# tencent-ailab/V-Express

Hardware: NVIDIA H100
Metric: frames_per_sec_512x512_25step (higher is better)
Workload: dtype bf16

## Files before the change

v-express_b200/csrc/vx_gemm.cu:

```cuda
#include "vx_host.h"
#include "vx_ptx.cuh"

namespace vx {

constexpr int kBlockM = 128;
constexpr int kBlockK = 64;
constexpr int kThreads = 384;
constexpr int kEpiThreads = 256;
constexpr int kPPMaxBN = 96;
constexpr int kPanelCols = 32;
constexpr int kPanelBytes = kBlockM * kPanelCols * 2;
constexpr int kSmemCap = 227 * 1024;
constexpr int kSmemReserve = 2048;

struct GemmArgs {
  int M, N;
  int kblocks1;
  int kblocks2;
  int taps;
  int rr;
  int a_bytes;
  int ups;
  int block_n;
  int pp;
  int stages;
  int nbuf;
  int rows_valid;
  int W, H;
  int cstride;
  int cpad;
  int tiles_m, tiles_n;
  int geglu;
  int has_residual;
  int out_f32;
  const float* bias;
  const float* bias2;
  int bias2_div;
  float scale;
  float* out32;
  long long ldc;
  const float* ln_stats;
  const float* ln_colsum;
  int ares;
  int ares_bytes;
  float2* rs_out;
  long long rs_stride;
  const float2* ln_parts;
  long long ln_pstride;
  int ln_nparts;
  float ln_invK;
  float ln_eps;
};

__device__ __forceinline__ void tma_store_2d(const CUtensorMap* m, const void* src, int c0, int c1) {
  asm volatile("cp.async.bulk.tensor.2d.global.shared::cta.bulk_group [%0, {%2, %3}], [%1];" ::"l"(
                   reinterpret_cast<uint64_t>(m)),
               "r"(smem_u32(src)), "r"(c0), "r"(c1)
               : "memory");
}
__device__ __forceinline__ void tma_store_5d(const CUtensorMap* m, const void* src, int c0, int c1, int c2, int c3, int c4) {
  asm volatile("cp.async.bulk.tensor.5d.global.shared::cta.bulk_group [%0, {%2, %3, %4, %5, %6}], [%1];" ::"l"(
                   reinterpret_cast<uint64_t>(m)),
// ... 45 lines not shown
  uint8_t* ring = smem;
  if constexpr (LNF) ring += p.ares ? p.ares_bytes : 0;
  uint8_t* sC = ring + p.stages * stage_bytes;
  const int out_cols = p.geglu ? BN / 2 : BN;
  const int npanels = out_cols / kPanelCols;
  const int buf_bytes = npanels * kPanelBytes;
  uint64_t* full_bar = reinterpret_cast<uint64_t*>(sC + (p.out_f32 ? 0 : p.nbuf * buf_bytes));
  uint64_t* empty_bar = full_bar + p.stages;
  uint64_t* c_ready = empty_bar + p.stages;
  uint64_t* staged = c_ready + 2;
  uint64_t* a_land = staged + 2;
  uint64_t* a_empty = a_land + 8;

  const int warp = threadIdx.x >> 5;
  const int lane = threadIdx.x & 31;
  const int total_kb = p.rr ? 3 * p.kblocks1 : p.taps * p.kblocks1 + p.kblocks2;
  const int tiles_per_par = p.tiles_m * p.tiles_n;
  const int num_tiles = tiles_per_par * (p.ups ? 4 : 1);
  auto item_at = [&](int it) -> int {
    if constexpr (LNF) {
      if (p.ares) {
        const int g = (int)blockIdx.x + (it / p.tiles_n) * (int)gridDim.x;
        return g < p.tiles_m ? g * p.tiles_n + it % p.tiles_n : -1;
      }
    }
    const int t = (int)blockIdx.x + it * (int)gridDim.x;
    return t < num_tiles ? t : -1;
  };

  if (threadIdx.x == 0) {
    tma_prefetch_desc(&mapA);
    tma_prefetch_desc(&mapB);
    if (p.kblocks2) tma_prefetch_desc(&mapA2);
    if (!p.out_f32) tma_prefetch_desc(&mapC);
    if (p.has_residual || p.ups) tma_prefetch_desc(&mapR);
    constexpr int consumers = PP ? kEpiThreads / 2 : kEpiThreads;
    for (int s = 0; s < p.stages; ++s) {
      mbar_init(&full_bar[s], 1);
      mbar_init(&empty_bar[s], consumers / 32);
    }
    for (int s = 0; s < 2; ++s) {
      mbar_init(&c_ready[s], 1);
      mbar_init(&staged[s], consumers);
    }
    for (int s = 0; s < 8; ++s) {
      mbar_init(&a_land[s], 1);
      mbar_init(&a_empty[s], kEpiThreads / 32);
    }
    fence_barrier_init();
  }
  __syncthreads();
  pdl_wait();

  if (warp < 4) setmaxnreg_dec<40>();
  else setmaxnreg_inc<232>();

  if (warp == 0) {
    const bool leader = elect_one();
    int stage = 0;
    uint32_t phase = 0;
    for (int it = 0, t = item_at(0); t >= 0; t = item_at(++it)) {
      const int par = t / tiles_per_par, tt = t - par * tiles_per_par;
      const int tile_n = tt % p.tiles_n, tile_m = tt / p.tiles_n;
      int n0 = 0, y0 = 0, x0 = 0;
      const long long m0 = (long long)tile_m * p.rows_valid;
      if (p.taps != 1) {
        const long long hw = (long long)p.H * p.W;
        n0 = (int)(m0 / hw);
        const int rem = (int)(m0 % hw);
        y0 = rem / p.W;
        x0 = rem % p.W;
      }
      const uint32_t tx_bytes = (uint32_t)((p.rr ? a_bytes : p.rows_valid * kBlockK * 2) + nbt * b_bytes);
      const int b_row = par * p.N + tile_n * BN;
      if constexpr (LNF) {
        if (p.ares && tile_n == 0) {
          for (int kb = 0; kb < p.kblocks1; ++kb) {
            mbar_wait(&a_empty[kb], (uint32_t)(((it / p.tiles_n) & 1) ^ 1));
            if (leader) {
              mbar_expect_tx(&a_land[kb], (uint32_t)(kBlockM * kBlockK * 2));
              tma_load_2d(smem + kb * (kBlockM * kBlockK * 2), &mapA, &a_land[kb], kb * kBlockK, (int)m0);
            }
          }
          __syncwarp();
        }
      }
      for (int kb = 0; kb < total_kb; ++kb) {
        mbar_wait(&empty_bar[stage], phase ^ 1);
        uint8_t* sa = ring + stage * stage_bytes;
        uint8_t* sb = sa + a_bytes;
        const int tap = p.taps != 1 ? kb / p.kblocks1 : 0;
        const int cb = kb - tap * p.kblocks1;
        if constexpr (LNF) {
          if (p.ares) {
            if (leader) {
              mbar_expect_tx(&full_bar[stage], (uint32_t)b_bytes);
              tma_load_2d(ring + stage * stage_bytes, &mapB, &full_bar[stage], kb * kBlockK, b_row);
            }
            __syncwarp();
            if (++stage == p.stages) {
              stage = 0;
              phase ^= 1;
            }
            continue;
          }
        }
        if (leader) {
          mbar_expect_tx(&full_bar[stage], tx_bytes);
          if (p.rr) {
            tma_load_4d(sa, &mapA, &full_bar[stage], cb * kBlockK, x0 + tap - 1, y0 - 1, n0);
#pragma unroll
            for (int dyi = 0; dyi < 3; ++dyi)
              tma_load_2d(sb + dyi * b_bytes, &mapB, &full_bar[stage], ((dyi * 3 + tap) * p.kblocks1 + cb) * kBlockK, b_row);
          } else {
            const int dy = p.ups ? (tap >> 1) + (par >> 1) - 1 : tap / 3 - p.cpad;
            const int dx = p.ups ? (tap & 1) + (par & 1) - 1 : tap % 3 - p.cpad;
            if (p.taps != 1) {
              tma_load_4d(sa, &mapA, &full_bar[stage], cb * kBlockK, x0 * p.cstride + dx, y0 * p.cstride + dy, n0);
            } else if (kb < p.kblocks1) {
              tma_load_2d(sa, &mapA, &full_bar[stage], kb * kBlockK, (int)m0);
            } else {
              tma_load_2d(sa, &mapA2, &full_bar[stage], (kb - p.kblocks1) * kBlockK, (int)m0);
            }
            tma_load_2d(sb, &mapB, &full_bar[stage], kb * kBlockK, b_row);
          }
        }
        __syncwarp();
        if (++stage == p.stages) {
          stage = 0;
          phase ^= 1;
        }
      }
    }
  } else if (warp == 1) {
    if (lane == 0 && !p.out_f32) {
      const uint32_t res_bytes = (uint32_t)(p.rows_valid * out_cols * 2);
      auto arm = [&](int t, int b) {
        if (p.has_residual) {
          const int tn_ = t % p.tiles_n, tm_ = t / p.tiles_n;
          mbar_expect_tx(&c_ready[b], res_bytes);
          for (int pn = 0; pn < npanels; ++pn)
            tma_load_2d(sC + b * buf_bytes + pn * kPanelBytes, &mapR, &c_ready[b], tn_ * out_cols + pn * kPanelCols,
                        tm_ * p.rows_valid);
        } else {
          mbar_arrive(&c_ready[b]);
        }
      };
      for (int b = 0; b < p.nbuf; ++b)
        if (item_at(b) >= 0) arm(item_at(b), b);
      for (int it = 0, t = item_at(0); t >= 0; t = item_at(++it)) {
        const int b = it % p.nbuf;
        const int par = t / tiles_per_par, tt = t - par * tiles_per_par;
        const int tile_n = tt % p.tiles_n, tile_m = tt / p.tiles_n;
        mbar_wait(&staged[b], (uint32_t)((it / p.nbuf) & 1));
        if (p.ups) {
          const long long m0 = (long long)tile_m * p.rows_valid, hw = (long long)p.H * p.W;
          const int n0 = (int)(m0 / hw), rem = (int)(m0 % hw);
          const CUtensorMap* mo = (par & 1) ? &mapR : &mapC;
          if (m0 < p.M)
            for (int pn = 0; pn < npanels; ++pn)
              tma_store_5d(mo, sC + b * buf_bytes + pn * kPanelBytes, tile_n * out_cols + pn * kPanelCols, rem % p.W,
                           rem / p.W, n0, par >> 1);
        } else {
          for (int pn = 0; pn < npanels; ++pn)
            tma_store_2d(&mapC, sC + b * buf_bytes + pn * kPanelBytes, tile_n * out_cols + pn * kPanelCols,
                         tile_m * p.rows_valid);
        }
        tma_store_commit();
        const int tnext = item_at(it + p.nbuf);
        if (tnext >= 0) {
          tma_store_wait_read();
          arm(tnext, b);
        }
      }
      tma_store_wait_all();
    }
  } else if (warp >= 4) {
    static_assert(!(PP && LNF) && (!PP || BN <= kPPMaxBN), "ping-pong: plain epilogues, BN <= 96");
    constexpr int MH = PP ? 2 : 1;
    const int wg = (threadIdx.x >> 7) - 1;
    const int wrow = (PP ? 0 : wg * 64) + (warp & 3) * 16 + (lane >> 2);
    const int cq = (lane & 3) * 2;
    float acc[MH][BN / 2];
#pragma unroll
    for (int mh = 0; mh < MH; ++mh)
#pragma unroll
      for (int i = 0; i < BN / 2; ++i) acc[mh][i] = 0.f;
    float ln_mean[2] = {0.f, 0.f}, ln_rstd[2] = {1.f, 1.f};
    for (int it = PP ? wg : 0, t = item_at(it); t >= 0; it += PP ? 2 : 1, t = item_at(it)) {
      const long long g0 = (long long)it * total_kb;
      int stage = (int)(g0 % p.stages);
      uint32_t phase = (uint32_t)((g0 / p.stages) & 1);
      if constexpr (PP) {
        if (it > 0) asm volatile("bar.sync %0, 256;" ::"r"(1 + wg) : "memory");
      }
      const int tt = t % tiles_per_par;
      const int tile_n = tt % p.tiles_n, tile_m = tt / p.tiles_n;
      bool a_last = false;
      if constexpr (LNF) {
        if (p.ares) {
          a_last = tile_n == p.tiles_n - 1;
          if (tile_n == 0) {
            const uint32_t a_phase = (uint32_t)((it / p.tiles_n) & 1);
            float s[2] = {0.f, 0.f};
            for (int kb = 0; kb < p.kblocks1; ++kb) {
              mbar_wait(&a_land[kb], a_phase);
#pragma unroll
              for (int h = 0; h < 2; ++h) {
                const uint8_t* rowp = smem + kb * (kBlockM * kBlockK * 2) + (wrow + 8 * h) * 128;
#pragma unroll
                for (int j = 0; j < 2; ++j) {
                  const uint4 q = *reinterpret_cast<const uint4*>(rowp + ((lane & 3) + 4 * j) * 16);
                  const uint32_t w[4] = {q.x, q.y, q.z, q.w};
#pragma unroll
                  for (int i = 0; i < 4; ++i) {
                    const float2 f2 = unpack_bf16(w[i]);
                    s[h] += f2.x + f2.y;
                  }
                }
              }
            }
            const float invK = 1.0f / (float)(p.kblocks1 * kBlockK);
#pragma unroll
            for (int h = 0; h < 2; ++h) ln_mean[h] = quad_sum(s[h]) * invK;
            float q2[2] = {0.f, 0.f};
            for (int kb = 0; kb < p.kblocks1; ++kb) {
#pragma unroll
              for (int h = 0; h < 2; ++h) {
                const uint8_t* rowp = smem + kb * (kBlockM * kBlockK * 2) + (wrow + 8 * h) * 128;
#pragma unroll
                for (int j = 0; j < 2; ++j) {
                  const uint4 q = *reinterpret_cast<const uint4*>(rowp + ((lane & 3) + 4 * j) * 16);
                  const uint32_t w[4] = {q.x, q.y, q.z, q.w};
#pragma unroll
                  for (int i = 0; i < 4; ++i) {
                    const float2 f2 = unpack_bf16(w[i]);
                    const float d0 = f2.x - ln_mean[h], d1 = f2.y - ln_mean[h];
                    q2[h] = fmaf(d0, d0, q2[h]);
                    q2[h] = fmaf(d1, d1, q2[h]);
                  }
                }
              }
            }
#pragma unroll
            for (int h = 0; h < 2; ++h) ln_rstd[h] = rsqrtf(quad_sum(q2[h]) * invK + p.ln_eps);
          }
        }
      }
      int prev = -1;
      for (int kb = 0; kb < total_kb; ++kb) {
        mbar_wait(&full_bar[stage], phase);
        uint32_t sa = smem_u32(ring + stage * stage_bytes);
        const uint32_t sb = sa + (uint32_t)a_bytes;
        if constexpr (LNF) {
          if (p.ares) sa = smem_u32(smem + kb * (kBlockM * kBlockK * 2));
        }
        if constexpr (!PP) sa += (uint32_t)(wg * 64 * 128);
        wgmma_fence();
        if (!PP && p.rr) {
#pragma unroll
          for (int dyi = 0; dyi < 3; ++dyi) {
            const uint64_t da = make_smem_desc(sa + (uint32_t)(dyi * p.W * 128), 16, 1024, SWZ_128B);
            const uint64_t db = make_smem_desc(sb + (uint32_t)(dyi * b_bytes), 16, 1024, SWZ_128B);
#pragma unroll
            for (int k = 0; k < kBlockK / 16; ++k)
              Wgmma<BN>::template ss<0, 0>(acc[0], da + (uint64_t)(k * 2), db + (uint64_t)(k * 2), (kb | dyi | k) != 0);
          }
        } else {
          const uint64_t db = make_smem_desc(sb, 16, 1024, SWZ_128B);
#pragma unroll
          for (int k = 0; k < kBlockK / 16; ++k)
#pragma unroll
            for (int mh = 0; mh < MH; ++mh) {
              const uint64_t da = make_smem_desc(sa + (uint32_t)(mh * 64 * 128), 16, 1024, SWZ_128B);
              Wgmma<BN>::template ss<0, 0>(acc[mh], da + (uint64_t)(k * 2), db + (uint64_t)(k * 2), (kb | k) != 0);
            }
        }
        wgmma_commit();
        wgmma_wait<1>();
        if (prev >= 0 && lane == 0) mbar_arrive(&empty_bar[prev]);
        prev = stage;
        if (++stage == p.stages) {
          stage = 0;
          phase ^= 1;
        }
      }
      if constexpr (PP) {
        if (item_at(it + 1) >= 0) asm volatile("bar.arrive %0, 256;" ::"r"(1 + (wg ^ 1)) : "memory");
      }
      wgmma_wait<0>();
#pragma unroll
      for (int mh = 0; mh < MH; ++mh) wgmma_fence_regs(acc[mh]);
      if (lane == 0) {
        mbar_arrive(&empty_bar[prev]);
        if constexpr (LNF) {
          if (a_last)
            for (int kb = 0; kb < p.kblocks1; ++kb) mbar_arrive(&a_empty[kb]);
        }
      }

      const int sb = it % p.nbuf;
      if (!p.out_f32) mbar_wait(&c_ready[sb], (uint32_t)((it / p.nbuf) & 1));
      uint8_t* buf = sC + sb * buf_bytes;
      const int nbase = tile_n * BN;
#pragma unroll
      for (int mh = 0; mh < MH; ++mh) {
        const int rbase = wrow + 64 * mh;
        float (&ac)[BN / 2] = acc[mh];
        long long m[2];
        bool row_ok[2];
        const float* b2[2];
#pragma unroll
        for (int h = 0; h < 2; ++h) {
          const int r = rbase + 8 * h;
          m[h] = (long long)tile_m * p.rows_valid + r;
          row_ok[h] = r < p.rows_valid && m[h] < p.M;
          b2[h] = p.bias2 ? p.bias2 + (row_ok[h] ? (m[h] / p.bias2_div) : 0) * (long long)p.N : nullptr;
          if constexpr (LNF) {
            if (p.ares) {
// ... 83 lines not shown
                const float2 t2 = unpack_bf16(pk);
                const int half = nl >= BN / 2;
                rs_sum[h][half] += t2.x + t2.y;
                rs_sq[h][half] = fmaf(t2.x, t2.x, fmaf(t2.y, t2.y, rs_sq[h][half]));
              }
            }
          }
          if (!PP && p.rs_out) {
#pragma unroll
            for (int h = 0; h < 2; ++h)
#pragma unroll
              for (int half = 0; half < 2; ++half) {
                const float s1 = quad_sum(rs_sum[h][half]), s2 = quad_sum(rs_sq[h][half]);
                if ((lane & 3) == 0 && row_ok[h]) p.rs_out[(long long)(tile_n * 2 + half) * p.rs_stride + m[h]] = make_float2(s1, s2);
              }
          }
        }
      }
      if (!p.out_f32) {
        fence_proxy_async_smem();
        mbar_arrive(&staged[sb]);
      }
    }
  }
}

struct GemmEnv {
  int stages, nbuf, bn, verbose, conv_rr, pp;
  static int geti(const char* name, int dflt) {
    const char* s = getenv(name);
    return s ? atoi(s) : dflt;
  }
  GemmEnv() {
    stages = geti("VX_GEMM_STAGES", 0);
    nbuf = geti("VX_GEMM_NBUF", 0);
    bn = geti("VX_GEMM_BN", 0);
    verbose = geti("VX_GEMM_VERBOSE", 0);
    conv_rr = geti("VX_CONV_RR", 1);
    pp = geti("VX_GEMM_PP", -1);
  }
};
static GemmEnv& gemm_env() {
  static GemmEnv e;
  return e;
}

static bool bn_supported(int bn) {
  switch (bn) {
    case 16: case 32: case 64: case 96: case 128: case 160: case 192: case 256: return true;
    default: return false;
  }
}

static bool pp_bn_supported(int bn) { return bn == 32 || bn == 64 || bn == 96; }

static int pick_block_n(long long tiles_m, int N, int gran, int total_kb, int fixed_bn = 0, bool pp_ok = false,
                        int* pp = nullptr) {
  const int mode = gemm_env().pp;
  if (pp) *pp = 0;
  if (pp_ok && mode != 0) {
    for (int bn = kPPMaxBN; bn >= 32; bn -= 32) {
      if (mode == -1 && bn != kPPMaxBN) break;
      if (N % bn || bn % gran || (fixed_bn > 0 && bn != fixed_bn)) continue;
      if (pp) *pp = 1;
      return bn;
    }
  }
  const int sms = device_sms();
  int best = 0;
  double best_cost = 1e30;
  for (int bn = 256; bn >= gran; bn -= gran) {
    if (N % bn || !bn_supported(bn) || (fixed_bn > 0 && bn != fixed_bn)) continue;
    const long long items = tiles_m * (N / bn);
    const double waves = (double)((items + sms - 1) / sms);
    const double cyc = (4.0 * bn > 128.0 + 2.0 * bn) ? 4.0 * bn : 128.0 + 2.0 * bn;
    const double cost = waves * (total_kb * (cyc + 40.0) + 4.0 * bn);
    if (cost < best_cost * 0.999) {
      best_cost = cost;
      best = bn;
    }
  }
  return best;
}

template <int BN, bool LNF, bool PP>
static cudaError_t launch_bn(const CUtensorMap& mA, const CUtensorMap& mA2, const CUtensorMap& mB, const CUtensorMap& mR,
                             const CUtensorMap& mC, const GemmArgs& a, int grid, size_t smem, cudaStream_t st) {
  static bool configured = false;
  if (!configured) {
    const cudaError_t e = cudaFuncSetAttribute(gemm_wgmma_kernel<BN, LNF, PP>, cudaFuncAttributeMaxDynamicSharedMemorySize, kSmemCap);
    if (e != cudaSuccess) return e;
    configured = true;
  }
  return launch_k((gemm_wgmma_kernel<BN, LNF, PP>), dim3(grid), dim3(kThreads), smem, st, mA, mA2, mB, mR, mC, a);
}

template <bool LNF>
static cudaError_t launch_lnf(const CUtensorMap& mA, const CUtensorMap& mA2, const CUtensorMap& mB, const CUtensorMap& mR,
                              const CUtensorMap& mC, const GemmArgs& a, int grid, size_t smem, cudaStream_t st) {
  if constexpr (!LNF) {
    if (a.pp) {
      switch (a.block_n) {
        case 32: return launch_bn<32, false, true>(mA, mA2, mB, mR, mC, a, grid, smem, st);
        case 64: return launch_bn<64, false, true>(mA, mA2, mB, mR, mC, a, grid, smem, st);
        case 96: return launch_bn<96, false, true>(mA, mA2, mB, mR, mC, a, grid, smem, st);
        default: return cudaErrorInvalidValue;
      }
    }
  }
  switch (a.block_n) {
    case 16: return launch_bn<16, LNF, false>(mA, mA2, mB, mR, mC, a, grid, smem, st);
    case 32: return launch_bn<32, LNF, false>(mA, mA2, mB, mR, mC, a, grid, smem, st);
    case 64: return launch_bn<64, LNF, false>(mA, mA2, mB, mR, mC, a, grid, smem, st);
    case 96: return launch_bn<96, LNF, false>(mA, mA2, mB, mR, mC, a, grid, smem, st);
    case 128: return launch_bn<128, LNF, false>(mA, mA2, mB, mR, mC, a, grid, smem, st);
    case 160: return launch_bn<160, LNF, false>(mA, mA2, mB, mR, mC, a, grid, smem, st);
    case 192: return launch_bn<192, LNF, false>(mA, mA2, mB, mR, mC, a, grid, smem, st);
    case 256: return launch_bn<256, LNF, false>(mA, mA2, mB, mR, mC, a, grid, smem, st);
    default: return cudaErrorInvalidValue;
  }
}

static int launch(const CUtensorMap& mA, const CUtensorMap& mA2, const CUtensorMap& mB, const CUtensorMap& mR,
                  const CUtensorMap& mC, GemmArgs& a, cudaStream_t st) {
  VX_REQUIRE(bn_supported(a.block_n), "vx_gemm: block_n=%d is not one of 16, 32, 64, 96, 128, 160, 192, 256", a.block_n);
  if (a.ares) a.a_bytes = 0;
  else if (a.a_bytes <= 0) a.a_bytes = kBlockM * kBlockK * 2;
  const int stage_bytes = a.a_bytes + (a.rr ? 3 : 1) * a.block_n * kBlockK * 2;
  const int out_cols = a.geglu ? a.block_n / 2 : a.block_n;
  const int buf_bytes = a.out_f32 ? 0 : out_cols / kPanelCols * kPanelBytes;
  const int total_kb = a.rr ? 3 * a.kblocks1 : a.taps * a.kblocks1 + a.kblocks2;
  const size_t cap = (size_t)kSmemCap - kSmemReserve - (a.ares ? (size_t)a.ares_bytes : 0);
  int want_stages = gemm_env().stages;
  if (want_stages <= 0) want_stages = total_kb < 6 ? (total_kb < 3 ? 3 : total_kb) : 6;
  int nbuf = (!a.out_f32 && (size_t)3 * stage_bytes + 2 * buf_bytes <= cap) ? 2 : 1;
  if (a.rr) {
    nbuf = ((size_t)3 * stage_bytes + buf_bytes <= cap) ? 1 : 2;
    want_stages = nbuf == 1 ? 3 : 2;
    if ((size_t)want_stages * stage_bytes + (size_t)nbuf * buf_bytes > cap) nbuf = 1;
  }
  if (a.ares) {
    nbuf = ((size_t)4 * stage_bytes + 2 * (size_t)buf_bytes <= cap) ? 2 : 1;
    want_stages = 8;
  }
  const int force_nbuf = gemm_env().nbuf;
  if (force_nbuf == 1 || (force_nbuf == 2 && (size_t)2 * stage_bytes + 2 * buf_bytes <= cap)) nbuf = force_nbuf;
  int stages = want_stages;
  while (stages > 2 && (size_t)stages * stage_bytes + (size_t)nbuf * buf_bytes > cap) --stages;
  a.stages = stages;
  a.nbuf = nbuf;
  if (a.pp && !a.out_f32 && nbuf != 2) a.pp = 0;
  const size_t smem = (size_t)stages * stage_bytes + (size_t)nbuf * buf_bytes + kSmemReserve + (a.ares ? (size_t)a.ares_bytes : 0);
  VX_REQUIRE(smem <= (size_t)kSmemCap, "vx_gemm: %zu bytes of shared memory needed (bn=%d, K blocks=%d)", smem, a.block_n,
             a.kblocks1);
  if (gemm_env().verbose)
    fprintf(stderr, "[vx_gemm] M=%d N=%d kb=%d taps=%d bn=%d pp=%d stages=%d nbuf=%d tiles=%dx%d\n", a.M, a.N, total_kb,
            a.taps, a.block_n, a.pp, stages, nbuf, a.tiles_m, a.tiles_n);
  const int npar = a.ups ? 4 : 1;
  const bool lnf = a.ln_stats != nullptr || a.ln_parts != nullptr || a.ares;
  VX_REQUIRE(!a.pp || (a.taps == 1 && !lnf && !a.rs_out && pp_bn_supported(a.block_n)), "vx_gemm: no ping-pong kernel for bn=%d",
             a.block_n);
  const long long tiles = a.ares ? a.tiles_m : (long long)a.tiles_m * a.tiles_n * npar;
  const int grid = tiles < device_sms() ? (int)tiles : device_sms();
  if (lnf) VX_CHECK_CUDA((launch_lnf<true>(mA, mA2, mB, mR, mC, a, grid, smem, st)));
  else VX_CHECK_CUDA((launch_lnf<false>(mA, mA2, mB, mR, mC, a, grid, smem, st)));
  VX_CHECK_CUDA(cudaGetLastError());
  return 0;
}

static int make_out_maps(CUtensorMap* mR, CUtensorMap* mC, const void* residual, long long ldr, void* out,
                         long long ldc, long long M, int out_N, int rows_valid) {
  uint64_t dims[2] = {(uint64_t)out_N, (uint64_t)M};
  uint32_t box[2] = {kPanelCols, (uint32_t)rows_valid};
  {
    uint64_t str[1] = {(uint64_t)ldc * 2};
    if (make_tmap_bf16(mC, out, 2, dims, str, box, CU_TENSOR_MAP_SWIZZLE_64B)) return 1;
  }
  if (residual) {
    uint64_t str[1] = {(uint64_t)ldr * 2};
    if (make_tmap_bf16(mR, residual, 2, dims, str, box, CU_TENSOR_MAP_SWIZZLE_64B)) return 1;
  } else {
    *mR = *mC;
  }
  return 0;
}

}

using namespace vx;

extern "C" void vx_gemm_reload_env() { gemm_env() = GemmEnv(); }

struct RowStatsIO {
  float* out;
  long long out_stride;
  int out_cap;
  int* nparts_out;
  const float* parts;
  long long parts_stride;
  int nparts;
};

static int gemm_entry(const void* A, long long lda, int K1, const void* A2, long long lda2, int K2, const void* Wt,
                      long long ldw, int M, int N, const float* bias, const float* bias2, int bias2_div, float scale,
                      const void* residual, long long ldr, void* out, long long ldc, int out_f32, int block_n,
                      const float* ln_stats, const float* ln_colsum, void* stream, float ln_eps = 0.f,
                      const RowStatsIO* rs = nullptr) {
  const int geglu = out_f32 == 2 ? 1 : 0;
  const bool ares = ln_colsum && !ln_stats && !(rs && rs->parts);
  if (geglu) out_f32 = 0;
  VX_REQUIRE(M > 0 && N > 0 && K1 > 0, "vx_gemm_bf16: bad shape M=%d N=%d K1=%d", M, N, K1);
  const int gran = geglu ? 64 : (out_f32 ? 16 : 32);
  VX_REQUIRE(N % gran == 0, "vx_gemm_bf16: N=%d must be a multiple of %d", N, gran);
  VX_REQUIRE(K1 % 8 == 0 && K2 % 8 == 0 && lda % 8 == 0 && ldw % 8 == 0 && ldc % 8 == 0,
// ... 128 lines not shown
}

extern "C" int vx_gemm_lnparts_bf16(const void* A, long long lda, int K, const void* Wt, long long ldw, int M, int N,
                                    const float* row_parts, long long parts_stride, int nparts, float eps,
                                    const float* colsum, const float* bias, const float* bias2, int bias2_div, float scale,
                                    const void* residual, long long ldr, void* out, long long ldc, int geglu, int block_n,
                                    void* stream) {
  VX_REQUIRE(row_parts && colsum, "vx_gemm_lnparts_bf16: row_parts / colsum missing (M=%d)", M);
  RowStatsIO rs{nullptr, 0, 0, nullptr, row_parts, parts_stride, nparts};
  return gemm_entry(A, lda, K, nullptr, 0, 0, Wt, ldw, M, N, bias, bias2, bias2_div, scale, residual, ldr, out, ldc,
                    geglu ? 2 : 0, block_n, nullptr, colsum, stream, eps, &rs);
}

extern "C" int vx_gemm_ln_bf16(const void* A, long long lda, int K, const void* Wt, long long ldw, int M, int N,
                               const float* colsum, const float* bias, float eps, const float* bias2, int bias2_div,
                               float scale, const void* residual, long long ldr, void* out, long long ldc, int geglu,
                               int block_n, void* stream) {
  VX_REQUIRE(colsum, "vx_gemm_ln_bf16: colsum missing (M=%d)", M);
  return gemm_entry(A, lda, K, nullptr, 0, 0, Wt, ldw, M, N, bias, bias2, bias2_div, scale, residual, ldr, out, ldc,
                    geglu ? 2 : 0, block_n, nullptr, colsum, stream, eps);
}

static int conv3x3_entry(const void* X, int NB, int Hin, int Win, int C, const void* Wt, int Cout, const float* bias,
                         const float* bias2, int bias2_div, float scale, const void* residual, long long ldr, void* out,
                         long long ldc, int block_n, int stride, int pad_lo, void* stream) {
  VX_REQUIRE(C % kBlockK == 0 && Cout % 32 == 0, "vx_conv3x3_bf16: C=%d must be %%64, Cout=%d %%32", C, Cout);
  VX_REQUIRE(ldc % 8 == 0 && (!residual || ldr % 8 == 0), "vx_conv3x3_bf16: ld must be %%8");
  VX_REQUIRE(stride == 1 || (stride == 2 && Hin % 2 == 0 && Win % 2 == 0), "vx_conv3x3: stride %d on %dx%d unsupported", stride,
             Hin, Win);
  VX_REQUIRE(pad_lo == 1 || (pad_lo == 0 && stride == 2), "vx_conv3x3: pad_lo=%d only with stride 2", pad_lo);
  const int H = Hin / stride, W = Win / stride;
  int wbox, hbox = 1, nbox = 1;
  if (W >= kBlockM) {
    wbox = kBlockM;
    while (W % wbox) --wbox;
  } else {
    wbox = W;
    hbox = kBlockM / W;
    if (hbox > H) {
      hbox = H;
      nbox = kBlockM / (W * H);
      if (nbox > NB) nbox = NB;
      if (nbox < 1) nbox = 1;
      while (NB % nbox) --nbox;
    } else {
      while (H % hbox) --hbox;
    }
  }
  const int rows_valid = wbox * hbox * nbox;
  const long long M = (long long)NB * H * W;
  VX_REQUIRE(M % rows_valid == 0, "vx_conv3x3_bf16: NB*H*W=%lld not tileable by %d", M, rows_valid);
  const long long tiles_m = M / rows_valid;
  const int total_kb = 9 * (C / kBlockK);
  if (block_n <= 0) block_n = gemm_env().bn;
  if (block_n <= 0) block_n = pick_block_n(tiles_m, Cout, 32, total_kb);
  VX_REQUIRE(block_n % 32 == 0 && block_n >= 32 && block_n <= 256 && Cout % block_n == 0,
             "vx_conv3x3_bf16: block_n=%d invalid for Cout=%d", block_n, Cout);
  bool rr = gemm_env().conv_rr && stride == 1 && nbox == 1 && wbox == W && hbox >= 2 && rows_valid == kBlockM && (W * 128) % 1024 == 0;
  if (rr) {
    const size_t st = (size_t)(hbox + 2) * W * kBlockK * 2 + (size_t)3 * block_n * kBlockK * 2;
    if (2 * st + (size_t)(block_n / kPanelCols) * kPanelBytes > (size_t)kSmemCap - kSmemReserve) rr = false;
  }
  CUtensorMap mA, mB, mR, mC;
  {
    uint64_t dims[4] = {(uint64_t)C, (uint64_t)Win, (uint64_t)Hin, (uint64_t)NB};
    uint64_t str[3] = {(uint64_t)C * 2, (uint64_t)Win * C * 2, (uint64_t)Hin * Win * C * 2};
    uint32_t box[4] = {kBlockK, (uint32_t)(wbox * stride), (uint32_t)((rr ? hbox + 2 : hbox) * stride), (uint32_t)nbox};
    uint32_t est[4] = {1, (uint32_t)stride, (uint32_t)stride, 1};
    if (make_tmap_bf16(&mA, X, 4, dims, str, box, CU_TENSOR_MAP_SWIZZLE_128B, est)) return 1;
  }
  {
    uint64_t dims[2] = {(uint64_t)9 * C, (uint64_t)Cout};
    uint64_t str[1] = {(uint64_t)9 * C * 2};
    uint32_t box[2] = {kBlockK, (uint32_t)block_n};
    if (make_tmap_bf16(&mB, Wt, 2, dims, str, box, CU_TENSOR_MAP_SWIZZLE_128B)) return 1;
  }
  if (make_out_maps(&mR, &mC, residual, ldr, out, ldc, M, Cout, rows_valid)) return 1;
  GemmArgs a{};
  a.M = (int)M; a.N = Cout;
  a.kblocks1 = C / kBlockK;
  a.kblocks2 = 0;
  a.taps = 9;
  a.rr = rr ? 1 : 0;
  a.a_bytes = rr ? (hbox + 2) * W * kBlockK * 2 : kBlockM * kBlockK * 2;
  a.block_n = block_n;
  a.rows_valid = rows_valid;
  a.W = W; a.H = H;
  a.cstride = stride; a.cpad = pad_lo;
  a.tiles_m = (int)tiles_m;
  a.tiles_n = Cout / block_n;
  a.geglu = 0;
  a.has_residual = residual ? 1 : 0;
  a.out_f32 = 0;
  a.bias = bias; a.bias2 = bias2; a.bias2_div = bias2_div > 0 ? bias2_div : 1; a.scale = scale;
  a.out32 = (float*)out; a.ldc = ldc;
  return launch(mA, mA, mB, mR, mC, a, (cudaStream_t)stream);
}

extern "C" int vx_conv3x3_bf16(const void* X, int NB, int H, int W, int C, const void* Wt, int Cout,
                               const float* bias, const float* bias2, int bias2_div, float scale,
                               const void* residual, long long ldr, void* out, long long ldc, int block_n,
                               void* stream) {
  return conv3x3_entry(X, NB, H, W, C, Wt, Cout, bias, bias2, bias2_div, scale, residual, ldr, out, ldc, block_n, 1, 1, stream);
}

extern "C" int vx_conv3x3s2_bf16(const void* X, int NB, int H, int W, int C, const void* Wt, int Cout, const float* bias,
                                 int pad_lo, void* out, long long ldc, int block_n, void* stream) {
  return conv3x3_entry(X, NB, H, W, C, Wt, Cout, bias, nullptr, 1, 1.0f, nullptr, 0, out, ldc, block_n, 2, pad_lo, stream);
}

extern "C" int vx_upconv3x3_bf16(const void* X, int NB, int H, int W, int C, const void* Wt, int Cout, const float* bias,
                                 void* out, long long ldc, int block_n, void* stream) {
  VX_REQUIRE(C % kBlockK == 0 && Cout % 32 == 0, "vx_upconv3x3_bf16: C=%d must be %%64, Cout=%d %%32", C, Cout);
  VX_REQUIRE(ldc % 8 == 0, "vx_upconv3x3_bf16: ldc must be %%8");
  int wbox, hbox = 1, nbox = 1;
  if (W >= kBlockM) {
    wbox = kBlockM;
    while (W % wbox) --wbox;
  } else {
    wbox = W;
    hbox = kBlockM / W;
    if (hbox > H) {
      hbox = H;
      nbox = kBlockM / (W * H);
      if (nbox > NB) nbox = NB;
      if (nbox < 1) nbox = 1;
      while (NB % nbox) --nbox;
    } else {
      while (H % hbox) --hbox;
    }
  }
  const int rows_valid = wbox * hbox * nbox;
  const long long M = (long long)NB * H * W;
  VX_REQUIRE(M % rows_valid == 0, "vx_upconv3x3_bf16: NB*H*W=%lld not tileable by %d", M, rows_valid);
  const long long tiles_m = M / rows_valid;
  const int total_kb = 4 * (C / kBlockK);
  if (block_n <= 0) block_n = gemm_env().bn;
  if (block_n <= 0) block_n = pick_block_n(tiles_m * 4, Cout, 32, total_kb);
  VX_REQUIRE(block_n % 32 == 0 && block_n >= 32 && block_n <= 256 && Cout % block_n == 0,
             "vx_upconv3x3_bf16: block_n=%d invalid for Cout=%d", block_n, Cout);
  CUtensorMap mA, mB, mC0, mC1;
  {
    uint64_t dims[4] = {(uint64_t)C, (uint64_t)W, (uint64_t)H, (uint64_t)NB};
    uint64_t str[3] = {(uint64_t)C * 2, (uint64_t)W * C * 2, (uint64_t)H * W * C * 2};
    uint32_t box[4] = {kBlockK, (uint32_t)wbox, (uint32_t)hbox, (uint32_t)nbox};
    if (make_tmap_bf16(&mA, X, 4, dims, str, box, CU_TENSOR_MAP_SWIZZLE_128B)) return 1;
  }
  {
    uint64_t dims[2] = {(uint64_t)4 * C, (uint64_t)4 * Cout};
    uint64_t str[1] = {(uint64_t)4 * C * 2};
    uint32_t box[2] = {kBlockK, (uint32_t)block_n};
    if (make_tmap_bf16(&mB, Wt, 2, dims, str, box, CU_TENSOR_MAP_SWIZZLE_128B)) return 1;
  }
  for (int px = 0; px < 2; ++px) {
    uint64_t dims[5] = {(uint64_t)Cout, (uint64_t)W, (uint64_t)H, (uint64_t)NB, 2};
    uint64_t str[4] = {(uint64_t)2 * ldc * 2, (uint64_t)2 * (2 * W) * ldc * 2, (uint64_t)(2 * H) * (2 * W) * ldc * 2,
                       (uint64_t)(2 * W) * ldc * 2};
    uint32_t box[5] = {kPanelCols, (uint32_t)wbox, (uint32_t)hbox, (uint32_t)nbox, 1};
    if (make_tmap_bf16(px ? &mC1 : &mC0, (const __nv_bfloat16*)out + (long long)px * ldc, 5, dims, str, box,
                       CU_TENSOR_MAP_SWIZZLE_64B))
      return 1;
  }
  GemmArgs a{};
  a.M = (int)M; a.N = Cout;
  a.kblocks1 = C / kBlockK;
  a.kblocks2 = 0;
  a.taps = 4;
  a.ups = 1;
  a.cstride = 1; a.cpad = 1;
  a.block_n = block_n;
  a.rows_valid = rows_valid;
  a.W = W; a.H = H;
  a.tiles_m = (int)tiles_m;
  a.tiles_n = Cout / block_n;
  a.geglu = 0;
  a.has_residual = 0;
  a.out_f32 = 0;
  a.bias = bias; a.bias2 = nullptr; a.bias2_div = 1; a.scale = 1.0f;
  a.out32 = (float*)out; a.ldc = ldc;
  return launch(mA, mA, mB, mC1, mC0, a, (cudaStream_t)stream);
}
```

Before: 5.266.

## Extend ping-pong warpgroup scheduling to conv3x3 and upconv kernels with wider tiles

Lets the ping-pong consumer schedule, where two warpgroups alternate tiles so one's epilogue overlaps the other's MMA, run on implicit-GEMM 3x3 convolutions, including the row-reuse path and the upsampling conv. It also allows block_n up to 160. A cost model in pick_block_n now weighs ping-pong against cooperative tiles using an assumed gain factor, and gates it on wave count and K depth. Stage and output-buffer sizing for the row-reuse path changes when ping-pong is on. The warp-role branches are nested under the register-reallocation split. Risks are higher register pressure from wider accumulators doubled per warpgroup, and shared-memory capacity limits.

Result: faster. 5.463 (median of 6 runs) (+3.7%).

```diff
diff --git a/v-express_b200/csrc/vx_gemm.cu b/v-express_b200/csrc/vx_gemm.cu
--- a/v-express_b200/csrc/vx_gemm.cu
+++ b/v-express_b200/csrc/vx_gemm.cu
@@ -7,7 +7,7 @@
 constexpr int kBlockK = 64;
 constexpr int kThreads = 384;
 constexpr int kEpiThreads = 256;
-constexpr int kPPMaxBN = 96;
+constexpr int kPPMaxBN = 160;
 constexpr int kPanelCols = 32;
 constexpr int kPanelBytes = kBlockM * kPanelCols * 2;
 constexpr int kSmemCap = 227 * 1024;
@@ -159,131 +159,132 @@
   __syncthreads();
   pdl_wait();
 
-  if (warp < 4) setmaxnreg_dec<40>();
-  else setmaxnreg_inc<232>();
-
-  if (warp == 0) {
-    const bool leader = elect_one();
-    int stage = 0;
-    uint32_t phase = 0;
-    for (int it = 0, t = item_at(0); t >= 0; t = item_at(++it)) {
-      const int par = t / tiles_per_par, tt = t - par * tiles_per_par;
-      const int tile_n = tt % p.tiles_n, tile_m = tt / p.tiles_n;
-      int n0 = 0, y0 = 0, x0 = 0;
-      const long long m0 = (long long)tile_m * p.rows_valid;
-      if (p.taps != 1) {
-        const long long hw = (long long)p.H * p.W;
-        n0 = (int)(m0 / hw);
-        const int rem = (int)(m0 % hw);
-        y0 = rem / p.W;
-        x0 = rem % p.W;
-      }
-      const uint32_t tx_bytes = (uint32_t)((p.rr ? a_bytes : p.rows_valid * kBlockK * 2) + nbt * b_bytes);
-      const int b_row = par * p.N + tile_n * BN;
-      if constexpr (LNF) {
-        if (p.ares && tile_n == 0) {
-          for (int kb = 0; kb < p.kblocks1; ++kb) {
-            mbar_wait(&a_empty[kb], (uint32_t)(((it / p.tiles_n) & 1) ^ 1));
-            if (leader) {
-              mbar_expect_tx(&a_land[kb], (uint32_t)(kBlockM * kBlockK * 2));
-              tma_load_2d(smem + kb * (kBlockM * kBlockK * 2), &mapA, &a_land[kb], kb * kBlockK, (int)m0);
-            }
-          }
-          __syncwarp();
+  if (warp < 4) {
+    setmaxnreg_dec<40>();
+    if (warp == 0) {
+      const bool leader = elect_one();
+      int stage = 0;
+      uint32_t phase = 0;
+      for (int it = 0, t = item_at(0); t >= 0; t = item_at(++it)) {
+        const int par = t / tiles_per_par, tt = t - par * tiles_per_par;
+        const int tile_n = tt % p.tiles_n, tile_m = tt / p.tiles_n;
+        int n0 = 0, y0 = 0, x0 = 0;
+        const long long m0 = (long long)tile_m * p.rows_valid;
+        if (p.taps != 1) {
+          const long long hw = (long long)p.H * p.W;
+          n0 = (int)(m0 / hw);
+          const int rem = (int)(m0 % hw);
+          y0 = rem / p.W;
+          x0 = rem % p.W;
         }
-      }
-      for (int kb = 0; kb < total_kb; ++kb) {
-        mbar_wait(&empty_bar[stage], phase ^ 1);
-        uint8_t* sa = ring + stage * stage_bytes;
-        uint8_t* sb = sa + a_bytes;
-        const int tap = p.taps != 1 ? kb / p.kblocks1 : 0;
-        const int cb = kb - tap * p.kblocks1;
+        const uint32_t tx_bytes = (uint32_t)((p.rr ? a_bytes : p.rows_valid * kBlockK * 2) + nbt * b_bytes);
+        const int b_row = par * p.N + tile_n * BN;
         if constexpr (LNF) {
-          if (p.ares) {
-            if (leader) {
-              mbar_expect_tx(&full_bar[stage], (uint32_t)b_bytes);
-              tma_load_2d(ring + stage * stage_bytes, &mapB, &full_bar[stage], kb * kBlockK, b_row);
+          if (p.ares && tile_n == 0) {
+            for (int kb = 0; kb < p.kblocks1; ++kb) {
+              mbar_wait(&a_empty[kb], (uint32_t)(((it / p.tiles_n) & 1) ^ 1));
+              if (leader) {
+                mbar_expect_tx(&a_land[kb], (uint32_t)(kBlockM * kBlockK * 2));
+                tma_load_2d(smem + kb * (kBlockM * kBlockK * 2), &mapA, &a_land[kb], kb * kBlockK, (int)m0);
+              }
             }
             __syncwarp();
-            if (++stage == p.stages) {
-              stage = 0;
-              phase ^= 1;
+          }
+        }
+        for (int kb = 0; kb < total_kb; ++kb) {
+          mbar_wait(&empty_bar[stage], phase ^ 1);
+          uint8_t* sa = ring + stage * stage_bytes;
+          uint8_t* sb = sa + a_bytes;
+          const int tap = p.taps != 1 ? kb / p.kblocks1 : 0;
+          const int cb = kb - tap * p.kblocks1;
+          if constexpr (LNF) {
+            if (p.ares) {
+              if (leader) {
+                mbar_expect_tx(&full_bar[stage], (uint32_t)b_bytes);
+                tma_load_2d(ring + stage * stage_bytes, &mapB, &full_bar[stage], kb * kBlockK, b_row);
+              }
+              __syncwarp();
+              if (++stage == p.stages) {
+                stage = 0;
+                phase ^= 1;
+              }
+              continue;
             }
-            continue;
+          }
+          if (leader) {
+            mbar_expect_tx(&full_bar[stage], tx_bytes);
+            if (p.rr) {
+              tma_load_4d(sa, &mapA, &full_bar[stage], cb * kBlockK, x0 + tap - 1, y0 - 1, n0);
+  #pragma unroll
+              for (int dyi = 0; dyi < 3; ++dyi)
+                tma_load_2d(sb + dyi * b_bytes, &mapB, &full_bar[stage], ((dyi * 3 + tap) * p.kblocks1 + cb) * kBlockK, b_row);
+            } else {
+              const int dy = p.ups ? (tap >> 1) + (par >> 1) - 1 : tap / 3 - p.cpad;
+              const int dx = p.ups ? (tap & 1) + (par & 1) - 1 : tap % 3 - p.cpad;
+              if (p.taps != 1) {
+                tma_load_4d(sa, &mapA, &full_bar[stage], cb * kBlockK, x0 * p.cstride + dx, y0 * p.cstride + dy, n0);
+              } else if (kb < p.kblocks1) {
+                tma_load_2d(sa, &mapA, &full_bar[stage], kb * kBlockK, (int)m0);
+              } else {
+                tma_load_2d(sa, &mapA2, &full_bar[stage], (kb - p.kblocks1) * kBlockK, (int)m0);
+              }
+              tma_load_2d(sb, &mapB, &full_bar[stage], kb * kBlockK, b_row);
+            }
+          }
+          __syncwarp();
+          if (++stage == p.stages) {
+            stage = 0;
+            phase ^= 1;
           }
         }
-        if (leader) {
-          mbar_expect_tx(&full_bar[stage], tx_bytes);
-          if (p.rr) {
-            tma_load_4d(sa, &mapA, &full_bar[stage], cb * kBlockK, x0 + tap - 1, y0 - 1, n0);
-#pragma unroll
-            for (int dyi = 0; dyi < 3; ++dyi)
-              tma_load_2d(sb + dyi * b_bytes, &mapB, &full_bar[stage], ((dyi * 3 + tap) * p.kblocks1 + cb) * kBlockK, b_row);
+      }
+    } else if (warp == 1) {
+      if (lane == 0 && !p.out_f32) {
+        const uint32_t res_bytes = (uint32_t)(p.rows_valid * out_cols * 2);
+        auto arm = [&](int t, int b) {
+          if (p.has_residual) {
+            const int tn_ = t % p.tiles_n, tm_ = t / p.tiles_n;
+            mbar_expect_tx(&c_ready[b], res_bytes);
+            for (int pn = 0; pn < npanels; ++pn)
+              tma_load_2d(sC + b * buf_bytes + pn * kPanelBytes, &mapR, &c_ready[b], tn_ * out_cols + pn * kPanelCols,
+                          tm_ * p.rows_valid);
           } else {
-            const int dy = p.ups ? (tap >> 1) + (par >> 1) - 1 : tap / 3 - p.cpad;
-            const int dx = p.ups ? (tap & 1) + (par & 1) - 1 : tap % 3 - p.cpad;
-            if (p.taps != 1) {
-              tma_load_4d(sa, &mapA, &full_bar[stage], cb * kBlockK, x0 * p.cstride + dx, y0 * p.cstride + dy, n0);
-            } else if (kb < p.kblocks1) {
-              tma_load_2d(sa, &mapA, &full_bar[stage], kb * kBlockK, (int)m0);
-            } else {
-              tma_load_2d(sa, &mapA2, &full_bar[stage], (kb - p.kblocks1) * kBlockK, (int)m0);
-            }
-            tma_load_2d(sb, &mapB, &full_bar[stage], kb * kBlockK, b_row);
+            mbar_arrive(&c_ready[b]);
+          }
+        };
+        for (int b = 0; b < p.nbuf; ++b)
+          if (item_at(b) >= 0) arm(item_at(b), b);
+        for (int it = 0, t = item_at(0); t >= 0; t = item_at(++it)) {
+          const int b = it % p.nbuf;
+          const int par = t / tiles_per_par, tt = t - par * tiles_per_par;
+          const int tile_n = tt % p.tiles_n, tile_m = tt / p.tiles_n;
+          mbar_wait(&staged[b], (uint32_t)((it / p.nbuf) & 1));
+          if (p.ups) {
+            const long long m0 = (long long)tile_m * p.rows_valid, hw = (long long)p.H * p.W;
+            const int n0 = (int)(m0 / hw), rem = (int)(m0 % hw);
+            const CUtensorMap* mo = (par & 1) ? &mapR : &mapC;
+            if (m0 < p.M)
+              for (int pn = 0; pn < npanels; ++pn)
+                tma_store_5d(mo, sC + b * buf_bytes + pn * kPanelBytes, tile_n * out_cols + pn * kPanelCols, rem % p.W,
+                             rem / p.W, n0, par >> 1);
+          } else {
+            for (int pn = 0; pn < npanels; ++pn)
+              tma_store_2d(&mapC, sC + b * buf_bytes + pn * kPanelBytes, tile_n * out_cols + pn * kPanelCols,
+                           tile_m * p.rows_valid);
+          }
+          tma_store_commit();
+          const int tnext = item_at(it + p.nbuf);
+          if (tnext >= 0) {
+            tma_store_wait_read();
+            arm(tnext, b);
           }
         }
-        __syncwarp();
-        if (++stage == p.stages) {
-          stage = 0;
-          phase ^= 1;
-        }
-      }
-    }
-  } else if (warp == 1) {
-    if (lane == 0 && !p.out_f32) {
-      const uint32_t res_bytes = (uint32_t)(p.rows_valid * out_cols * 2);
-      auto arm = [&](int t, int b) {
-        if (p.has_residual) {
-          const int tn_ = t % p.tiles_n, tm_ = t / p.tiles_n;
-          mbar_expect_tx(&c_ready[b], res_bytes);
-          for (int pn = 0; pn < npanels; ++pn)
-            tma_load_2d(sC + b * buf_bytes + pn * kPanelBytes, &mapR, &c_ready[b], tn_ * out_cols + pn * kPanelCols,
-                        tm_ * p.rows_valid);
-        } else {
-          mbar_arrive(&c_ready[b]);
-        }
-      };
-      for (int b = 0; b < p.nbuf; ++b)
-        if (item_at(b) >= 0) arm(item_at(b), b);
-      for (int it = 0, t = item_at(0); t >= 0; t = item_at(++it)) {
-        const int b = it % p.nbuf;
-        const int par = t / tiles_per_par, tt = t - par * tiles_per_par;
-        const int tile_n = tt % p.tiles_n, tile_m = tt / p.tiles_n;
-        mbar_wait(&staged[b], (uint32_t)((it / p.nbuf) & 1));
-        if (p.ups) {
-          const long long m0 = (long long)tile_m * p.rows_valid, hw = (long long)p.H * p.W;
-          const int n0 = (int)(m0 / hw), rem = (int)(m0 % hw);
-          const CUtensorMap* mo = (par & 1) ? &mapR : &mapC;
-          if (m0 < p.M)
-            for (int pn = 0; pn < npanels; ++pn)
-              tma_store_5d(mo, sC + b * buf_bytes + pn * kPanelBytes, tile_n * out_cols + pn * kPanelCols, rem % p.W,
-                           rem / p.W, n0, par >> 1);
-        } else {
-          for (int pn = 0; pn < npanels; ++pn)
-            tma_store_2d(&mapC, sC + b * buf_bytes + pn * kPanelBytes, tile_n * out_cols + pn * kPanelCols,
-                         tile_m * p.rows_valid);
-        }
-        tma_store_commit();
-        const int tnext = item_at(it + p.nbuf);
-        if (tnext >= 0) {
-          tma_store_wait_read();
-          arm(tnext, b);
-        }
-      }
-      tma_store_wait_all();
-    }
-  } else if (warp >= 4) {
-    static_assert(!(PP && LNF) && (!PP || BN <= kPPMaxBN), "ping-pong: plain epilogues, BN <= 96");
+        tma_store_wait_all();
+      }
+    }
+  } else {
+    setmaxnreg_inc<232>();
+    static_assert(!(PP && LNF) && (!PP || BN <= kPPMaxBN), "ping-pong: plain epilogues, BN <= 160");
     constexpr int MH = PP ? 2 : 1;
     const int wg = (threadIdx.x >> 7) - 1;
     const int wrow = (PP ? 0 : wg * 64) + (warp & 3) * 16 + (lane >> 2);
@@ -364,14 +365,17 @@
         }
         if constexpr (!PP) sa += (uint32_t)(wg * 64 * 128);
         wgmma_fence();
-        if (!PP && p.rr) {
+        if (p.rr) {
 #pragma unroll
           for (int dyi = 0; dyi < 3; ++dyi) {
-            const uint64_t da = make_smem_desc(sa + (uint32_t)(dyi * p.W * 128), 16, 1024, SWZ_128B);
             const uint64_t db = make_smem_desc(sb + (uint32_t)(dyi * b_bytes), 16, 1024, SWZ_128B);
 #pragma unroll
             for (int k = 0; k < kBlockK / 16; ++k)
-              Wgmma<BN>::template ss<0, 0>(acc[0], da + (uint64_t)(k * 2), db + (uint64_t)(k * 2), (kb | dyi | k) != 0);
+#pragma unroll
+              for (int mh = 0; mh < MH; ++mh) {
+                const uint64_t da = make_smem_desc(sa + (uint32_t)(dyi * p.W * 128 + mh * 64 * 128), 16, 1024, SWZ_128B);
+                Wgmma<BN>::template ss<0, 0>(acc[mh], da + (uint64_t)(k * 2), db + (uint64_t)(k * 2), (kb | dyi | k) != 0);
+              }
           }
         } else {
           const uint64_t db = make_smem_desc(sb, 16, 1024, SWZ_128B);
@@ -561,34 +565,46 @@
   }
 }
 
-static bool pp_bn_supported(int bn) { return bn == 32 || bn == 64 || bn == 96; }
+static bool pp_bn_supported(int bn) { return bn == 32 || bn == 64 || bn == 96 || bn == 128 || bn == 160; }
+
+constexpr double kPPGain = 1.12;
+constexpr int kPPMaxKBlocks = 20;
 
 static int pick_block_n(long long tiles_m, int N, int gran, int total_kb, int fixed_bn = 0, bool pp_ok = false,
-                        int* pp = nullptr) {
+                        int* pp = nullptr, int pp_max_bn = kPPMaxBN, bool pp_any_k = false) {
   const int mode = gemm_env().pp;
+  auto fits = [&](int bn) { return N % bn == 0 && bn % gran == 0 && bn_supported(bn) && (fixed_bn <= 0 || bn == fixed_bn); };
   if (pp) *pp = 0;
-  if (pp_ok && mode != 0) {
-    for (int bn = kPPMaxBN; bn >= 32; bn -= 32) {
-      if (mode == -1 && bn != kPPMaxBN) break;
-      if (N % bn || bn % gran || (fixed_bn > 0 && bn != fixed_bn)) continue;
-      if (pp) *pp = 1;
-      return bn;
-    }
-  }
+  pp_ok = pp_ok && pp && mode != 0;
+  if (pp_ok && mode == 1) {
+    for (int bn = kPPMaxBN; bn >= 32; bn -= 32)
+      if (fits(bn) && pp_bn_supported(bn) && bn <= pp_max_bn) {
+        *pp = 1;
+        return bn;
+      }
+  }
+  if (!pp_any_k && total_kb > kPPMaxKBlocks) pp_ok = false;
   const int sms = device_sms();
-  int best = 0;
+  int best = 0, best_pp = 0;
   double best_cost = 1e30;
   for (int bn = 256; bn >= gran; bn -= gran) {
-    if (N % bn || !bn_supported(bn) || (fixed_bn > 0 && bn != fixed_bn)) continue;
+    if (!fits(bn)) continue;
     const long long items = tiles_m * (N / bn);
-    const double waves = (double)((items + sms - 1) / sms);
+    const long long waves = (items + sms - 1) / sms;
     const double cyc = (4.0 * bn > 128.0 + 2.0 * bn) ? 4.0 * bn : 128.0 + 2.0 * bn;
-    const double cost = waves * (total_kb * (cyc + 40.0) + 4.0 * bn);
+    const double cost = (double)waves * (total_kb * (cyc + 40.0) + 4.0 * bn);
     if (cost < best_cost * 0.999) {
       best_cost = cost;
       best = bn;
-    }
-  }
+      best_pp = 0;
+    }
+    if (pp_ok && pp_bn_supported(bn) && bn <= pp_max_bn && waves >= 2 && cost / kPPGain < best_cost * 0.999) {
+      best_cost = cost / kPPGain;
+      best = bn;
+      best_pp = 1;
+    }
+  }
+  if (pp) *pp = best_pp;
   return best;
 }
 
@@ -613,6 +629,8 @@
         case 32: return launch_bn<32, false, true>(mA, mA2, mB, mR, mC, a, grid, smem, st);
         case 64: return launch_bn<64, false, true>(mA, mA2, mB, mR, mC, a, grid, smem, st);
         case 96: return launch_bn<96, false, true>(mA, mA2, mB, mR, mC, a, grid, smem, st);
+        case 128: return launch_bn<128, false, true>(mA, mA2, mB, mR, mC, a, grid, smem, st);
+        case 160: return launch_bn<160, false, true>(mA, mA2, mB, mR, mC, a, grid, smem, st);
         default: return cudaErrorInvalidValue;
       }
     }
@@ -644,9 +662,9 @@
   if (want_stages <= 0) want_stages = total_kb < 6 ? (total_kb < 3 ? 3 : total_kb) : 6;
   int nbuf = (!a.out_f32 && (size_t)3 * stage_bytes + 2 * buf_bytes <= cap) ? 2 : 1;
   if (a.rr) {
-    nbuf = ((size_t)3 * stage_bytes + buf_bytes <= cap) ? 1 : 2;
-    want_stages = nbuf == 1 ? 3 : 2;
-    if ((size_t)want_stages * stage_bytes + (size_t)nbuf * buf_bytes > cap) nbuf = 1;
+    nbuf = (a.pp || (size_t)3 * stage_bytes + buf_bytes > cap) ? 2 : 1;
+    want_stages = nbuf == 1 || a.pp ? 3 : 2;
+    if (!a.pp && (size_t)want_stages * stage_bytes + (size_t)nbuf * buf_bytes > cap) nbuf = 1;
   }
   if (a.ares) {
     nbuf = ((size_t)4 * stage_bytes + 2 * (size_t)buf_bytes <= cap) ? 2 : 1;
@@ -663,12 +681,11 @@
   VX_REQUIRE(smem <= (size_t)kSmemCap, "vx_gemm: %zu bytes of shared memory needed (bn=%d, K blocks=%d)", smem, a.block_n,
              a.kblocks1);
   if (gemm_env().verbose)
-    fprintf(stderr, "[vx_gemm] M=%d N=%d kb=%d taps=%d bn=%d pp=%d stages=%d nbuf=%d tiles=%dx%d\n", a.M, a.N, total_kb,
-            a.taps, a.block_n, a.pp, stages, nbuf, a.tiles_m, a.tiles_n);
+    fprintf(stderr, "[vx_gemm] M=%d N=%d kb=%d taps=%d bn=%d pp=%d rr=%d stages=%d nbuf=%d tiles=%dx%d\n", a.M, a.N,
+            total_kb, a.taps, a.block_n, a.pp, a.rr, stages, nbuf, a.tiles_m, a.tiles_n);
   const int npar = a.ups ? 4 : 1;
   const bool lnf = a.ln_stats != nullptr || a.ln_parts != nullptr || a.ares;
-  VX_REQUIRE(!a.pp || (a.taps == 1 && !lnf && !a.rs_out && pp_bn_supported(a.block_n)), "vx_gemm: no ping-pong kernel for bn=%d",
-             a.block_n);
+  VX_REQUIRE(!a.pp || (!lnf && !a.rs_out && pp_bn_supported(a.block_n)), "vx_gemm: no ping-pong kernel for bn=%d", a.block_n);
   const long long tiles = a.ares ? a.tiles_m : (long long)a.tiles_m * a.tiles_n * npar;
   const int grid = tiles < device_sms() ? (int)tiles : device_sms();
   if (lnf) VX_CHECK_CUDA((launch_lnf<true>(mA, mA2, mB, mR, mC, a, grid, smem, st)));
@@ -903,15 +920,24 @@
   VX_REQUIRE(M % rows_valid == 0, "vx_conv3x3_bf16: NB*H*W=%lld not tileable by %d", M, rows_valid);
   const long long tiles_m = M / rows_valid;
   const int total_kb = 9 * (C / kBlockK);
+  bool rr = gemm_env().conv_rr && stride == 1 && nbox == 1 && wbox == W && hbox >= 2 && rows_valid == kBlockM && (W * 128) % 1024 == 0;
+  auto rr_fits = [&](int bn, int stages, int nbuf) {
+    const size_t st = (size_t)(hbox + 2) * W * kBlockK * 2 + (size_t)3 * bn * kBlockK * 2;
+    return stages * st + (size_t)nbuf * (bn / kPanelCols) * kPanelBytes <= (size_t)kSmemCap - kSmemReserve;
+  };
   if (block_n <= 0) block_n = gemm_env().bn;
-  if (block_n <= 0) block_n = pick_block_n(tiles_m, Cout, 32, total_kb);
+  int pp = 0;
+  {
+    const int fixed = block_n;
+    const int coop_bn = pick_block_n(tiles_m, Cout, 32, total_kb, fixed);
+    rr = rr && coop_bn > 0 && rr_fits(coop_bn, 2, 1);
+    int pp_max_bn = kPPMaxBN;
+    while (rr && pp_max_bn > 0 && !rr_fits(pp_max_bn, 3, 2)) pp_max_bn -= 32;
+    block_n = pick_block_n(tiles_m, Cout, 32, total_kb, fixed, true, &pp, pp_max_bn, rr);
+    if (!block_n) block_n = fixed;
+  }
   VX_REQUIRE(block_n % 32 == 0 && block_n >= 32 && block_n <= 256 && Cout % block_n == 0,
              "vx_conv3x3_bf16: block_n=%d invalid for Cout=%d", block_n, Cout);
-  bool rr = gemm_env().conv_rr && stride == 1 && nbox == 1 && wbox == W && hbox >= 2 && rows_valid == kBlockM && (W * 128) % 1024 == 0;
-  if (rr) {
-    const size_t st = (size_t)(hbox + 2) * W * kBlockK * 2 + (size_t)3 * block_n * kBlockK * 2;
-    if (2 * st + (size_t)(block_n / kPanelCols) * kPanelBytes > (size_t)kSmemCap - kSmemReserve) rr = false;
-  }
   CUtensorMap mA, mB, mR, mC;
   {
     uint64_t dims[4] = {(uint64_t)C, (uint64_t)Win, (uint64_t)Hin, (uint64_t)NB};
@@ -935,6 +961,7 @@
   a.rr = rr ? 1 : 0;
   a.a_bytes = rr ? (hbox + 2) * W * kBlockK * 2 : kBlockM * kBlockK * 2;
   a.block_n = block_n;
+  a.pp = pp;
   a.rows_valid = rows_valid;
   a.W = W; a.H = H;
   a.cstride = stride; a.cpad = pad_lo;
@@ -987,7 +1014,12 @@
   const long long tiles_m = M / rows_valid;
   const int total_kb = 4 * (C / kBlockK);
   if (block_n <= 0) block_n = gemm_env().bn;
-  if (block_n <= 0) block_n = pick_block_n(tiles_m * 4, Cout, 32, total_kb);
+  int pp = 0;
+  {
+    const int fixed = block_n;
+    block_n = pick_block_n(tiles_m * 4, Cout, 32, total_kb, fixed, true, &pp);
+    if (!block_n) block_n = fixed;
+  }
   VX_REQUIRE(block_n % 32 == 0 && block_n >= 32 && block_n <= 256 && Cout % block_n == 0,
              "vx_upconv3x3_bf16: block_n=%d invalid for Cout=%d", block_n, Cout);
   CUtensorMap mA, mB, mC0, mC1;
@@ -1020,6 +1052,7 @@
   a.ups = 1;
   a.cstride = 1; a.cpad = 1;
   a.block_n = block_n;
+  a.pp = pp;
   a.rows_valid = rows_valid;
   a.W = W; a.H = H;
   a.tiles_m = (int)tiles_m;
```
